# Anonymousijcai2024ttnet/scale_imagenet

Hardware: AMD Instinct MI355X
Metric: images/sec ImageNet 224x224, TT-small, MI355X; top-1 exact-match (higher is better)
Workload: dtype u16/u32/u64 packed bits (gate path); f32 as prescaled fp16x2 split operands on the 16-bit MFMA (stem, lin1, lin2); 1 GPU; TT_general_imagenet_v2_small forward, batch=256 224x224 per GPU, bit-packed HIP LUT kernels (BASELINE.json configs[1]); batch_per_gpu=256, global_batch=256, batches_in_flight=2, input=float32 NCHW, normalised (the reference's contract), parallelism=batch shard x1

## Files before the change

scale_imagenet_amd/csrc/gate_fused.hip:

```cpp

#include <type_traits>

#include "ttnet_common.h"

namespace ttnet {

namespace {

#ifndef TT_FUSED_SKIP
#define TT_FUSED_SKIP 0
#endif
constexpr int kSkip = TT_FUSED_SKIP;

constexpr int kFT = 1024;
constexpr int kFBuf = 65536;
constexpr int kFMaxScratch = 160 * 1024 - 2 * kFBuf;

template <int W>
using row_t = std::conditional_t<(W > 32), uint64_t, std::conditional_t<(W > 16), uint32_t, uint16_t>>;

template <int HO>
constexpr int fused_round() {
  constexpr int RG = (HO + 3) / 4, a = kFT / (16 * RG), b = kFMaxScratch / (HO * HO * 4);
  return a < b ? (a < 32 ? a : 32) : (b < 32 ? b : 32);
}

struct FusedArgs {
  int n, C, slices, off34, R;
  const void *x;
  const uint8_t *img_c3;
  const uint8_t *img_dw;
  const uint8_t *t_cf;
  void *y;
  uint32_t *idx;
};

__device__ inline void dma_table(uint8_t *dst, const uint8_t *src) {
  if constexpr (kSkip & 1) return;
  const int lane = threadIdx.x & 63, wave = threadIdx.x >> 6;
#pragma unroll
  for (int k = 0; k < kFBuf / 1024 / (kFT / 64); ++k) {
    const int chunk = wave + k * (kFT / 64);
    __builtin_amdgcn_global_load_lds((const __attribute__((address_space(1))) void *)(src + (size_t)chunk * 1024 + lane * 16),
                                     (__attribute__((address_space(3))) void *)(dst + chunk * 1024), 16, 0, 0);
  }
}

__device__ inline void phase_sync() {
  asm volatile("s_waitcnt vmcnt(0)" ::: "memory");
  __syncthreads();
}

__device__ inline uint32_t spread_nibbles(uint32_t x) {
  uint32_t y = (x | (x << 8)) & 0x00FF00FFu;
  return (y | (y << 4)) & 0x0F0F0F0Fu;
}

template <int WO, int OX0, int OX1>
__device__ inline void dw_lookup_pair(uint32_t pair, const uint8_t *tab, uint32_t c8, uint32_t &acc1, uint32_t &acc2) {
  if constexpr (OX0 < WO) {
    const uint2 w = *(const uint2 *)(tab + ((pair & 0xFFE0u) | c8));
    acc1 |= __builtin_amdgcn_ubfe(w.x, pair, 1) << OX0;
    acc2 |= __builtin_amdgcn_ubfe(w.y, pair, 1) << OX0;
  }
  if constexpr (OX1 < WO) {
    const uint32_t hi = pair >> 16;
    const uint2 w = *(const uint2 *)(tab + ((hi & 0xFFE0u) | c8));
    acc1 |= __builtin_amdgcn_ubfe(w.x, hi, 1) << OX1;
    acc2 |= __builtin_amdgcn_ubfe(w.y, hi, 1) << OX1;
  }
}

template <int WO, int OXB, int OXS>
__device__ inline void dw_eight(uint32_t R0, uint32_t R1, uint32_t R2, uint32_t R3, const uint8_t *tab, uint32_t c8,
                                uint32_t &acc1, uint32_t &acc2) {
  if constexpr (OXB >= WO) return;
  constexpr uint32_t M = 0x0F0F0F0Fu;
  const uint32_t t0 = (R0 & M) | ((R1 << 4) & ~M), u0 = (R2 & M) | ((R3 << 4) & ~M);
  dw_lookup_pair<WO, OXB, OXB + 2 * OXS>(__builtin_amdgcn_perm(u0, t0, 0x05010400u), tab, c8, acc1, acc2);
  dw_lookup_pair<WO, OXB + 4 * OXS, OXB + 6 * OXS>(__builtin_amdgcn_perm(u0, t0, 0x07030602u), tab, c8, acc1, acc2);
  if constexpr (OXB + OXS < WO) {
    const uint32_t t1 = ((R0 >> 4) & M) | (R1 & ~M), u1 = ((R2 >> 4) & M) | (R3 & ~M);
    dw_lookup_pair<WO, OXB + OXS, OXB + 3 * OXS>(__builtin_amdgcn_perm(u1, t1, 0x05010400u), tab, c8, acc1, acc2);
    dw_lookup_pair<WO, OXB + 5 * OXS, OXB + 7 * OXS>(__builtin_amdgcn_perm(u1, t1, 0x07030602u), tab, c8, acc1, acc2);
  }
}

template <int W, int WO>
__device__ inline void dw_row_both(const row_t<W> (&r)[4], const uint8_t *tab, uint32_t c8, uint32_t &acc1, uint32_t &acc2) {
  acc1 = 0;
  acc2 = 0;
  if constexpr (W > 32) {
    uint32_t plo[4], phi[4], qlo[4], qhi[4];
#pragma unroll
    for (int k = 0; k < 4; ++k) {
      qlo[k] = (uint32_t)r[k];
      qhi[k] = (uint32_t)((uint64_t)r[k] >> 32);
      plo[k] = qlo[k] << 2;
      phi[k] = __builtin_amdgcn_alignbit(qhi[k], qlo[k], 30);
    }
    dw_eight<WO, 0, 2>(plo[0], plo[1], plo[2], plo[3], tab, c8, acc1, acc2);
    dw_eight<WO, 16, 2>(phi[0], phi[1], phi[2], phi[3], tab, c8, acc1, acc2);
    dw_eight<WO, 1, 2>(qlo[0], qlo[1], qlo[2], qlo[3], tab, c8, acc1, acc2);
    dw_eight<WO, 17, 2>(qhi[0], qhi[1], qhi[2], qhi[3], tab, c8, acc1, acc2);
  } else {
    uint32_t p[4], q[4];
#pragma unroll
    for (int k = 0; k < 4; ++k) {
      q[k] = (uint32_t)r[k];
      p[k] = q[k] << 2;
    }
    dw_eight<WO, 0, 2>(p[0], p[1], p[2], p[3], tab, c8, acc1, acc2);
    dw_eight<WO, 1, 2>(q[0], q[1], q[2], q[3], tab, c8, acc1, acc2);
    static_assert(WO <= 16, "a 32-bit input row gives at most 16 output columns");
  }
}

__device__ inline uint32_t maj4_bytes(uint32_t v, uint32_t nb) {
  const uint32_t x = v & nb, y = v | nb;
  return (x | (x >> 8) | (y & (y >> 8))) & 0x00FF00FFu;
}

template <int H, int HO, bool LAST>
__global__ __launch_bounds__(kFT) void gate_block_kernel(FusedArgs a) {
  extern __shared__ __align__(16) uint8_t lds[];
  constexpr int W = H, WO = HO, HP = H / 2, WP = W / 2, PIX = HO * WO;
  constexpr int RG = (HO + 3) / 4;
  constexpr int LPR = WO <= 16 ? 16 : 32, RPW = 64 / LPR;
  using TI = row_t<W>;
  using TOut = row_t<WO>;
  uint8_t *const buf0 = lds, *const buf1 = lds + kFBuf;
  uint32_t *const S = (uint32_t *)(lds + 2 * kFBuf);

  const int strands = a.C / 8, P = strands / 2;
  int st, sl;
  {
    const int b = blockIdx.x, x = b & 7, k = b >> 3;
    if (P >= 8 && P % 8 == 0) {
      const int m = P / 8, pair = x + 8 * (k % m), kk = k / m;
      st = 2 * pair + (kk & 1);
      sl = kk >> 1;
    } else if (P == 4 && (a.slices & 1) == 0) {
      st = 2 * (x >> 1) + (k & 1);
      sl = (x & 1) * (a.slices / 2) + (k >> 1);
    } else {
      st = b % strands;
      sl = b / strands;
    }
  }
  const int n0 = (int)((long long)sl * a.n / a.slices), n1 = (int)((long long)(sl + 1) * a.n / a.slices);
  if (n0 >= n1) return;
  const int q = st >> 1, half = st & 1;
  const int tid0 = threadIdx.x, lane = tid0 & 63;
  const DwLaneConst lk = dw_lane_const(lane);
  auto opaque_tid = [&]() {
    int t = tid0;
    asm volatile("" : "+v"(t));
    return t;
  };
  const TI *const x = (const TI *)a.x;

  const uint8_t *const src_c3 = a.img_c3 + (size_t)st * kFBuf;
  const uint8_t *const src_dw0 = a.img_dw + (size_t)(2 * st) * kFBuf, *const src_dw1 = src_dw0 + kFBuf;
  const uint8_t *const src_cf0 = LAST ? nullptr : a.t_cf + (size_t)(2 * st) * kFBuf, *const src_cf1 = LAST ? nullptr : src_cf0 + kFBuf;

  constexpr int RMAX = fused_round<HO>();
  constexpr int TA = (RMAX * HP + kFT / 16 - 1) / (kFT / 16);
  static_assert(RMAX * RG * 16 <= kFT, "one depthwise task per thread");
  TI ra[TA][2];
  TI rb0[4], rb1[4];
  const int R = a.R;

  auto load_a = [&](int i0, int rn) {
    const int tid = opaque_tid();
    const int c = tid & 15, g = tid >> 4;
#pragma unroll
    for (int p = 0; p < TA; ++p) {
      const int gt = p * (kFT / 16) + g;
      const bool ok = gt < rn * HP;
      const int im = ok ? gt / HP : 0, py = ok ? gt - (gt / HP) * HP : 0;
      const TI *src = x + ((size_t)(n0 + i0 + im) * a.C + 16 * q + c) * H + 2 * py;
      ra[p][0] = ok ? src[0] : (TI)0;
      ra[p][1] = ok ? src[1] : (TI)0;
    }
  };
  auto load_b = [&](int i0, int rn, int sub, TI (&rb)[4]) {
    const int tid = opaque_tid();
    const int c4 = tid & 3, r = (tid >> 2) & 3, gi = tid >> 4;
    const int im = gi / RG, rg = gi - im * RG;
    const int oy = 4 * rg + r;
    const bool ok = im < rn && oy < HO;
    const TI *src = x + ((size_t)(n0 + i0 + (ok ? im : 0)) * a.C + 8 * st + 4 * sub + c4) * H;
#pragma unroll
    for (int kh = 0; kh < 4; ++kh) {
      const int iy = 2 * oy - 2 + kh;
      rb[kh] = (ok && iy >= 0 && iy < H) ? src[iy] : (TI)0;
    }
  };

  auto phase_a = [&](int rn, const uint8_t *tab) {
    if constexpr (kSkip & 2) return;
    const int tid = opaque_tid();
    for (int t = tid; t < rn * (HO + WO - 1); t += kFT) {
      const int im = t / (HO + WO - 1), e = t - im * (HO + WO - 1);
      const int edge = a.off34 ? 0 : HO - 1;
      const int pix = e < WO ? edge * WO + e : (e - WO + (a.off34 ? 1 : 0)) * WO + edge;
      *(uint16_t *)((uint8_t *)(S + im * PIX + pix) + 2) = 0;
    }
    const int g = tid >> 4, j = tid & 15;
    constexpr int CHUNKS = W > 32 ? 2 : 1, TPB = 2 / CHUNKS;
    static_assert(TA % TPB == 0, "phase A walks whole batches");
#pragma unroll
    for (int bt = 0; bt < TA / TPB; ++bt) {
      uint32_t d[4];
#pragma unroll
      for (int u = 0; u < 2; ++u) {
        const int p = bt * TPB + (CHUNKS == 2 ? 0 : u), k = CHUNKS == 2 ? u : 0;
        d[2 * u] = (uint32_t)((uint64_t)ra[p][0] >> (32 * k));
        d[2 * u + 1] = (uint32_t)((uint64_t)ra[p][1] >> (32 * k));
      }
      transpose16_multi<4>(d, lk);
      uint32_t v3[2], v4[2];
#pragma unroll
      for (int u = 0; u < 2; ++u) {
        const uint32_t t0 = d[2 * u], t1 = d[2 * u + 1];
        const uint32_t e00 = tab[t0 & 0xFFFFu], e01 = tab[t0 >> 16], e10 = tab[t1 & 0xFFFFu], e11 = tab[t1 >> 16];
        v3[u] = e00 | (e10 << 8) | (e01 << 16) | (e11 << 24);
        v4[u] = __builtin_amdgcn_perm(t1, t0, half ? 0x07030501u : 0x06020400u);
      }
      uint32_t n3[2], n4[2];
#pragma unroll
      for (int u = 0; u < 2; ++u) {
        n3[u] = lane_xor16<1>(v3[u]);
        n4[u] = lane_xor16<1>(v4[u]);
      }
#pragma unroll
      for (int u = 0; u < 2; ++u) {
        const int p = bt * TPB + (CHUNKS == 2 ? 0 : u), k = CHUNKS == 2 ? u : 0;
        const int gt = p * (kFT / 16) + g;
        const bool ok = gt < rn * HP;
        const int im = ok ? gt / HP : 0, py = ok ? gt - (gt / HP) * HP : 0;
        const uint32_t m3 = maj4_bytes(v3[u], n3[u]), m4 = maj4_bytes(v4[u], n4[u]);
        const uint32_t sh = (uint32_t)(j & 1) * 16u;
        const uint32_t t = ((m3 >> sh) & 0xFFu) | (((m4 >> sh) & 0xFFu) << 8);
        const uint32_t dlt = ((t >> 4) ^ t) & 0x00F0u;
        const uint32_t v = t ^ dlt ^ (dlt << 4);
        const int px = 16 * k + 8 * (j & 1) + (j >> 1);
        if (ok && px < WP) {
          const int pix = (py + a.off34) * WO + px + a.off34;
          *(uint16_t *)((uint8_t *)(S + im * PIX + pix) + 2) = (uint16_t)v;
        }
      }
      __builtin_amdgcn_sched_barrier(0);
    }
  };

  uint32_t bacc[2][2];
  auto phase_b_lookup = [&](const uint8_t *tab, int sub, const TI (&rb)[4]) {
    if constexpr (kSkip & 4) return;
    const int tid = opaque_tid();
    dw_row_both<W, WO>(rb, tab, (uint32_t)(tid & 3) * 8u, bacc[sub][0], bacc[sub][1]);
  };
  auto phase_b_store = [&](int rn) {
    if constexpr (kSkip & 4) return;
    const int tid = opaque_tid();
    const int j = tid & 15, gi = tid >> 4;
    const int im = gi / RG, rg = gi - im * RG;
    uint32_t t[4] = {bacc[0][0], bacc[0][1], bacc[1][0], bacc[1][1]};
    transpose16_multi<4>(t, lk);
    uint8_t *dst = (uint8_t *)(S + im * PIX + 4 * rg * WO + j);
    auto put = [&](uint32_t w0, uint32_t w1, int col0) {
      if (im < rn && col0 + j < WO) {
        const uint32_t lo = __builtin_amdgcn_perm(w1, w0, 0x05010400u), hi = __builtin_amdgcn_perm(w1, w0, 0x07030602u);
        if (4 * rg + 0 < HO) *(uint16_t *)(dst + (0 * WO + col0) * 4) = (uint16_t)lo;
        if (4 * rg + 1 < HO) *(uint16_t *)(dst + (1 * WO + col0) * 4) = (uint16_t)(lo >> 16);
        if (4 * rg + 2 < HO) *(uint16_t *)(dst + (2 * WO + col0) * 4) = (uint16_t)hi;
        if (4 * rg + 3 < HO) *(uint16_t *)(dst + (3 * WO + col0) * 4) = (uint16_t)(hi >> 16);
      }
    };
    put(spread_nibbles(t[0] & 0xFFFFu) | (spread_nibbles(t[1] & 0xFFFFu) << 4),
        spread_nibbles(t[2] & 0xFFFFu) | (spread_nibbles(t[3] & 0xFFFFu) << 4), 0);
    if constexpr (WO > 16)
      put(spread_nibbles(t[0] >> 16) | (spread_nibbles(t[1] >> 16) << 4), spread_nibbles(t[2] >> 16) | (spread_nibbles(t[3] >> 16) << 4), 16);
  };

  auto phase_c = [&](int i0, int rn, const uint8_t *tab, int kgrp) {
    if constexpr (kSkip & 8) return;
    const int tid = opaque_tid();
    const int lane = tid & 63, wave = __builtin_amdgcn_readfirstlane(tid >> 6);
    const int sub = lane / LPR, ox = lane % LPR;
    TOut *const y = (TOut *)a.y;
    constexpr int CH2 = (HO + 2 * RPW - 1) / (2 * RPW);
    constexpr int U = 2, NW = kFT / 64;
    const uint32_t sel = kgrp ? 0x0C0C0301u : 0x0C0C0200u;
    if (kgrp == 0 && a.idx)
      for (int t = tid; t < rn * PIX; t += kFT) a.idx[((size_t)(n0 + i0 + t / PIX) * strands + st) * PIX + (t % PIX)] = S[t];
    for (int wt0 = wave; wt0 < rn * CH2; wt0 += U * NW) {
      uint32_t w[U], d0[U], d1[U];
      int im[U], oy[U];
#pragma unroll
      for (int u = 0; u < U; ++u) {
        const int wt = wt0 + u * NW;
        im[u] = wt / CH2;
        oy[u] = (wt - im[u] * CH2) * 2 * RPW + sub;
        const bool live = wt < rn * CH2 && ox < WO;
        d0[u] = live && oy[u] < HO ? S[im[u] * PIX + oy[u] * WO + ox] : 0u;
        d1[u] = live && oy[u] + RPW < HO ? S[im[u] * PIX + (oy[u] + RPW) * WO + ox] : 0u;
      }
#pragma unroll
      for (int u = 0; u < U; ++u)
        w[u] = ox < WO ? (uint32_t)tab[__builtin_amdgcn_perm(0u, d0[u], sel)] | ((uint32_t)tab[__builtin_amdgcn_perm(0u, d1[u], sel)] << 8)
                       : 0u;
      transpose16_multi<U>(w, lk);
#pragma unroll
      for (int u = 0; u < U; ++u) {
        const uint32_t piece = w[u] & 0xFFFFu;
        uint32_t rowbits = piece;
        if constexpr (LPR == 32) rowbits |= (uint32_t)__shfl_xor((int)piece, 16) << 16;
        const int row = oy[u] + ((lane >> 3) & 1) * RPW;
        if (wt0 + u * NW < rn * CH2 && (lane & (LPR - 1)) < 16 && row < HO)
          y[((uint32_t)(n0 + i0 + im[u]) * (uint32_t)(2 * a.C) + 16 * st + 8 * kgrp + (lane & 7)) * HO + row] = (TOut)rowbits;
      }
    }
  };

  auto phase_out = [&](int i0, int rn) {
    const int tid = opaque_tid();
    for (int t = tid; t < rn * PIX; t += kFT)
      a.idx[((size_t)(n0 + i0 + t / PIX) * strands + st) * PIX + (t % PIX)] = S[t];
  };

  const int total = n1 - n0;
  int cur = 0;
  load_a(0, min(R, total));
  dma_table(buf0, src_c3);
  for (int i0 = 0; i0 < total; i0 += R) {
    const int rn = min(R, total - i0);
    const bool more = i0 + R < total;
    uint8_t *tb = cur ? buf1 : buf0, *nb = cur ? buf0 : buf1;
    phase_sync();
    load_b(i0, rn, 0, rb0);
    dma_table(nb, src_dw0);
    phase_a(rn, tb);
    cur ^= 1; tb = cur ? buf1 : buf0; nb = cur ? buf0 : buf1;
    phase_sync();
    load_b(i0, rn, 1, rb1);
    dma_table(nb, src_dw1);
    phase_b_lookup(tb, 0, rb0);
    cur ^= 1; tb = cur ? buf1 : buf0; nb = cur ? buf0 : buf1;
    phase_sync();
    if constexpr (LAST) {
      if (more) {
        load_a(i0 + R, min(R, total - i0 - R));
        dma_table(nb, src_c3);
      }
      phase_b_lookup(tb, 1, rb1);
      phase_b_store(rn);
      cur ^= 1;
      phase_sync();
      phase_out(i0, rn);
    } else {
      dma_table(nb, src_cf0);
      phase_b_lookup(tb, 1, rb1);
      phase_b_store(rn);
      cur ^= 1; tb = cur ? buf1 : buf0; nb = cur ? buf0 : buf1;
      phase_sync();
      dma_table(nb, src_cf1);
      phase_c(i0, rn, tb, 0);
      cur ^= 1; tb = cur ? buf1 : buf0; nb = cur ? buf0 : buf1;
      phase_sync();
      if (more) {
        load_a(i0 + R, min(R, total - i0 - R));
        dma_table(nb, src_c3);
      }
      phase_c(i0, rn, tb, 1);
      cur ^= 1;
    }
  }
}

__global__ void c3_image_kernel(const uint16_t *__restrict__ t_c3, uint8_t *__restrict__ img, int strands) {
  const size_t t = (size_t)blockIdx.x * blockDim.x + threadIdx.x;
  if (t >= (size_t)strands * 65536) return;
  const int st = (int)(t >> 16);
  const uint32_t idx = (uint32_t)(t & 0xFFFF);
  img[t] = (uint8_t)(t_c3[(size_t)(st >> 1) * 65536 + idx] >> (8 * (st & 1)));
}
__global__ void dw_image_kernel(const uint32_t *__restrict__ t1, const uint32_t *__restrict__ t2, uint32_t *__restrict__ img, int C) {
  const size_t t = (size_t)blockIdx.x * blockDim.x + threadIdx.x;
  if (t >= (size_t)C * 2048 * 2) return;
  const int br = (int)(t & 1), ch = (int)((t >> 1) & 3), row = (int)((t >> 3) & 2047), ss = (int)(t >> 14);
  const int channel = 4 * ss + ch;
  const uint32_t *src = br ? t2 : t1;
  img[t] = src[((size_t)(channel >> 4) * 2048 + row) * 16 + (channel & 15)];
}

__global__ void branch_rows_kernel(const uint32_t *__restrict__ idx, uint64_t *__restrict__ rows, int n, int C, int HO, int br) {
  const size_t t = (size_t)blockIdx.x * blockDim.x + threadIdx.x;
  if (t >= (size_t)n * C * HO) return;
  const int oy = (int)(t % HO), c = (int)((t / HO) % C), im = (int)(t / ((size_t)HO * C));
  const int st = c >> 3, k = c & 7;
  const int shift = 8 * ((br >> 1) * 2 + (k >> 2)) + 4 * (br & 1) + (k & 3);
  const uint32_t *src = idx + ((size_t)im * (C / 8) + st) * HO * HO + (size_t)oy * HO;
  uint64_t r = 0;
  for (int ox = 0; ox < HO; ++ox) r |= (uint64_t)((src[ox] >> shift) & 1u) << ox;
  rows[t] = r;
}
template <typename T>
__global__ void widen_rows_kernel(const T *__restrict__ src, uint64_t *__restrict__ dst, size_t count) {
  const size_t t = (size_t)blockIdx.x * blockDim.x + threadIdx.x;
  if (t < count) dst[t] = (uint64_t)src[t];
}
template <typename T>
__global__ void narrow_rows_kernel(const uint64_t *__restrict__ src, T *__restrict__ dst, size_t count) {
  const size_t t = (size_t)blockIdx.x * blockDim.x + threadIdx.x;
  if (t < count) dst[t] = (T)src[t];
}

template <int H, int HO, bool LAST>
int launch_block_t(const FusedBlockArgs &f, hipStream_t s) {
  auto k = gate_block_kernel<H, HO, LAST>;
  constexpr int PIX = HO * HO;
  const int strands = f.C / 8;
  int R = fused_round<HO>();
  const int slices = fused_block_slices(f.C, f.n);
  R = std::max(1, std::min(R, (f.n + slices - 1) / slices));
  const size_t lds = (size_t)2 * kFBuf + (size_t)R * PIX * 4;
  TT_TRY(ensure_dynamic_lds((const void *)k, kMaxLds));
  FusedArgs a{};
  a.n = f.n; a.C = f.C; a.slices = slices; a.off34 = f.off34; a.R = R;
  a.x = f.x; a.img_c3 = (const uint8_t *)f.img_c3; a.img_dw = (const uint8_t *)f.img_dw; a.t_cf = f.t_cf; a.y = f.y; a.idx = f.idx;
  hipLaunchKernelGGL(k, dim3(strands * slices), dim3(kFT), lds, s, a);
  TT_HIP(hipGetLastError());
  return TTNET_OK;
}

}

int row_bytes(int W) { return W > 32 ? 8 : (W > 16 ? 4 : 2); }

int fused_block_slices(int C, int n) {
  const int strands = C / 8;
  int slices = std::max(1, std::min(n, 256 / strands));
  if (strands == 8 && slices > 1 && (slices & 1)) slices -= 1;
  return slices;
}

bool fused_block_supported(int C, int H, int Ho, int stride, int pad, int kh, int kw) {
  if (stride != 2 || pad != 2 || kh != 4 || kw != 4 || C % 16) return false;
  return (H == 56 && Ho == 29) || (H == 29 && Ho == 15) || (H == 15 && Ho == 8) || (H == 8 && Ho == 5);
}

int launch_gate_block(const FusedBlockArgs &f, hipStream_t s) {
  if (f.last && !f.idx) {
    set_error("gate_block: a last block needs its branch-dword buffer");
    return TTNET_E_INVALID;
  }
#define TT_FUSED_CASE(h, ho)                                                         \
  if (f.H == h && f.Ho == ho) return f.last ? launch_block_t<h, ho, true>(f, s) : launch_block_t<h, ho, false>(f, s)
  if (f.H == 56 && f.Ho == 29 && !f.last) return launch_block_t<56, 29, false>(f, s);
  TT_FUSED_CASE(29, 15);
  TT_FUSED_CASE(15, 8);
  TT_FUSED_CASE(8, 5);
#undef TT_FUSED_CASE
  set_error("gate_block: no fused kernel for %dx%d -> %dx%d", f.H, f.H, f.Ho, f.Ho);
  return TTNET_E_UNSUPPORTED;
}

int launch_fused_images(const void *t_dw1, const void *t_dw2, const void *t_c3, int C, void *img_dw, void *img_c3, hipStream_t s) {
  {
    const size_t t = (size_t)(C / 8) * 65536;
    hipLaunchKernelGGL(c3_image_kernel, dim3((unsigned)((t + 255) / 256)), dim3(256), 0, s, (const uint16_t *)t_c3, (uint8_t *)img_c3,
                       C / 8);
  }
  {
    const size_t t = (size_t)C * 2048 * 2;
    hipLaunchKernelGGL(dw_image_kernel, dim3((unsigned)((t + 255) / 256)), dim3(256), 0, s, (const uint32_t *)t_dw1,
                       (const uint32_t *)t_dw2, (uint32_t *)img_dw, C);
  }
  TT_HIP(hipGetLastError());
  return TTNET_OK;
}

int launch_branch_rows(const uint32_t *idx, uint64_t *rows, int n, int C, int Ho, int branch, hipStream_t s) {
  const size_t t = (size_t)n * C * Ho;
  hipLaunchKernelGGL(branch_rows_kernel, dim3((unsigned)((t + 255) / 256)), dim3(256), 0, s, idx, rows, n, C, Ho, branch);
  TT_HIP(hipGetLastError());
  return TTNET_OK;
}

int launch_widen_rows(const void *src, uint64_t *dst, size_t count, int W, hipStream_t s) {
  const unsigned g = (unsigned)((count + 255) / 256);
  if (W > 32) hipLaunchKernelGGL(widen_rows_kernel<uint64_t>, dim3(g), dim3(256), 0, s, (const uint64_t *)src, dst, count);
  else if (W > 16) hipLaunchKernelGGL(widen_rows_kernel<uint32_t>, dim3(g), dim3(256), 0, s, (const uint32_t *)src, dst, count);
  else hipLaunchKernelGGL(widen_rows_kernel<uint16_t>, dim3(g), dim3(256), 0, s, (const uint16_t *)src, dst, count);
  TT_HIP(hipGetLastError());
  return TTNET_OK;
}

int launch_narrow_rows(const uint64_t *src, void *dst, size_t count, int W, hipStream_t s) {
  const unsigned g = (unsigned)((count + 255) / 256);
  if (W > 32) hipLaunchKernelGGL(narrow_rows_kernel<uint64_t>, dim3(g), dim3(256), 0, s, src, (uint64_t *)dst, count);
  else if (W > 16) hipLaunchKernelGGL(narrow_rows_kernel<uint32_t>, dim3(g), dim3(256), 0, s, src, (uint32_t *)dst, count);
  else hipLaunchKernelGGL(narrow_rows_kernel<uint16_t>, dim3(g), dim3(256), 0, s, src, (uint16_t *)dst, count);
  TT_HIP(hipGetLastError());
  return TTNET_OK;
}

}
```

scale_imagenet_amd/csrc/ttnet_common.h:

```cpp
#pragma once

#include <hip/hip_runtime.h>
#include <stdint.h>
#include <algorithm>
#include <string>
#include <type_traits>
#include <vector>

#include "../../include/ttnet.h"

namespace ttnet {

void set_error(const char *fmt, ...);

#define TT_HIP(call)                                                                       \
  do {                                                                                     \
    hipError_t e__ = (call);                                                               \
    if (e__ != hipSuccess) {                                                               \
      ::ttnet::set_error("%s failed: %s (%s:%d)", #call, hipGetErrorString(e__), __FILE__, \
                         __LINE__);                                                        \
      return TTNET_E_HIP;                                                                  \
    }                                                                                      \
  } while (0)

#define TT_TRY(expr)          \
  do {                        \
    int s__ = (expr);         \
    if (s__ != TTNET_OK) return s__; \
  } while (0)

constexpr int kWave = 64;
constexpr int kMaxLds = 160 * 1024;

struct BlockGeom {
  std::string name;
  int in_planes = 0, out_planes = 0, kh = 1, kw = 1, stride = 1, pad = 0, groups = 1;
  bool last = false;
  int cin_g() const { return in_planes / groups; }
  int mid_g() const { return 8 * in_planes / groups; }
  int cout_g() const { return out_planes / groups; }
  int nbits() const { return cin_g() * kh * kw; }
  int entry_bits() const { return last ? 32 * cout_g() : (cout_g() == 1 ? 1 : (cout_g() <= 8 ? 8 : 16)); }
  size_t table_bytes() const {
    size_t entries = (size_t)groups << nbits();
    if (last) return entries * cout_g() * sizeof(float);
    if (entry_bits() == 1) {
      const size_t per = ((size_t)1 << nbits()) / 8;
      return (size_t)groups * (per < 4 ? 4 : per);
    }
    return entries * entry_bits() / 8;
  }
};

#if defined(__HIPCC__)
template <int LANE>
__device__ inline void writelane64(uint32_t &lo, uint32_t &hi, uint64_t sval) {
  asm("s_nop 1\n\tv_writelane_b32 %0, %2, %4\n\tv_writelane_b32 %1, %3, %4"
      : "+v"(lo), "+v"(hi)
      : "s"((uint32_t)sval), "s"((uint32_t)(sval >> 32)), "n"(LANE));
}

template <int I, int N, typename F>
__device__ inline void static_for(F &&f) {
  if constexpr (I < N) {
    f(std::integral_constant<int, I>{});
    static_for<I + 1, N>(f);
  }
}

struct DwLaneConst {
  uint32_t c4;
  uint32_t rot[4];
  uint32_t keep[4];
};

__device__ inline DwLaneConst dw_lane_const(uint32_t lane) {
  DwLaneConst k;
  k.c4 = (lane & 15) << 2;
  constexpr uint32_t M[4] = {0x00FF00FFu, 0x0F0F0F0Fu, 0x33333333u, 0x55555555u};
  constexpr uint32_t S[4] = {8, 4, 2, 1};
#pragma unroll
  for (int i = 0; i < 4; ++i) {
    const bool low = (lane & S[i]) == 0;
    k.rot[i] = low ? 32 - S[i] : S[i];
    k.keep[i] = low ? M[i] : ~M[i];
  }
  return k;
}

__device__ inline uint32_t transpose16(uint32_t acc, const DwLaneConst &k) {
  constexpr int S[4] = {8, 4, 2, 1};
  static_for<0, 4>([&](auto i) {
    constexpr int I = decltype(i)::value;
    const uint32_t partner = (uint32_t)__builtin_amdgcn_ds_swizzle((int)acc, 0x1F | (S[I] << 10));
    const uint32_t moved = __builtin_amdgcn_alignbit(partner, partner, k.rot[I]);
    acc = moved ^ ((moved ^ acc) & k.keep[I]);
  });
  return acc;
}

template <int S>
__device__ inline uint32_t lane_xor16(uint32_t v) {
  static_assert(S == 8 || S == 4 || S == 2 || S == 1, "butterfly distances");
  if constexpr (S == 8) return (uint32_t)__builtin_amdgcn_mov_dpp((int)v, 0x128, 0xF, 0xF, true);
  else if constexpr (S == 4)
    return (uint32_t)__builtin_amdgcn_mov_dpp(__builtin_amdgcn_mov_dpp((int)v, 0x141, 0xF, 0xF, true), 0x1B, 0xF, 0xF, true);
  else if constexpr (S == 2) return (uint32_t)__builtin_amdgcn_mov_dpp((int)v, 0x4E, 0xF, 0xF, true);
  else return (uint32_t)__builtin_amdgcn_mov_dpp((int)v, 0xB1, 0xF, 0xF, true);
}

template <int N>
__device__ inline void transpose16_multi(uint32_t (&acc)[N], const DwLaneConst &k) {
  constexpr int S[4] = {8, 4, 2, 1};
  static_for<0, 4>([&](auto i) {
    constexpr int I = decltype(i)::value;
    uint32_t partner[N];
#pragma unroll
    for (int n = 0; n < N; ++n) partner[n] = lane_xor16<S[I]>(acc[n]);
#pragma unroll
    for (int n = 0; n < N; ++n) {
      const uint32_t moved = __builtin_amdgcn_alignbit(partner[n], partner[n], k.rot[I]);
      acc[n] = moved ^ ((moved ^ acc[n]) & k.keep[I]);
    }
  });
}

#endif

int ensure_dynamic_lds(const void *kernel, size_t bytes);


struct LutBuildArgs {
  const float *w1;
  const float *w2;
  const double *s1, *t1;
  const double *s2, *t2;
  const uint8_t *perm;
  int groups, n, mid_g, cout_g, last;
  void *table;
  unsigned *near_ties;
};
int launch_lut_build(const LutBuildArgs &a, hipStream_t s);

constexpr int SPLIT_PLANES = 2;
constexpr float ACT_PRESCALE = 16.0f;

__device__ inline void split_f16x2(float v, uint16_t &h1, uint16_t &h2) {
  const _Float16 a = (_Float16)v;
  const _Float16 b = (_Float16)(v - (float)a);
  h1 = __builtin_bit_cast(uint16_t, a);
  h2 = __builtin_bit_cast(uint16_t, b);
}
__device__ inline float f16_bits_to_float(uint16_t h) { return (float)__builtin_bit_cast(_Float16, h); }

__device__ inline bool split_out_of_range(float prescaled) { return !(__builtin_fabsf(prescaled) < 65504.0f); }

__device__ inline void store_feature(uint16_t *feat_frag, int img, int KS, int ks, int kk, float f, uint32_t *range_flag) {
  uint16_t h1, h2;
  const float fs = f * ACT_PRESCALE;
  if (split_out_of_range(fs)) *range_flag = 1u;
  split_f16x2(fs, h1, h2);
  const int ln = (img & 31) + 32 * (kk >> 3), j = kk & 7;
  const size_t base = ((size_t)(img >> 5) * KS + ks) * SPLIT_PLANES;
  feat_frag[((base + 0) * 64 + ln) * 8 + j] = h1;
  feat_frag[((base + 1) * 64 + ln) * 8 + j] = h2;
}
__device__ inline float load_feature(const uint16_t *feat_frag, int img, int KS, int ks, int kk) {
  const int ln = (img & 31) + 32 * (kk >> 3), j = kk & 7;
  const size_t base = ((size_t)(img >> 5) * KS + ks) * SPLIT_PLANES;
  return (f16_bits_to_float(feat_frag[((base + 1) * 64 + ln) * 8 + j]) + f16_bits_to_float(feat_frag[((base + 0) * 64 + ln) * 8 + j])) *
         (1.0f / ACT_PRESCALE);
}
float weight_prescale(const float *w, size_t n);

int launch_stem(const void *x, bool x_is_u8, const uint32_t *norm_tab, const void *wfrag, const float *init, uint64_t *rp,
                uint16_t *cp, int n, int p, uint32_t *range_flag, hipStream_t s, int workgroups = 0);
size_t stem_u8_table_elems();
bool stem_split_weights_u8(const float *w, const double *scale, const double *shift, int p, const float mean[3], const float stdv[3],
                           uint16_t *out, float *init, uint32_t *tab );
bool stem_split_weights(const float *w , const double *scale, const double *shift, int p, uint16_t *out,
                        float *init );
size_t stem_split_weights_elems();
int stem_kernel_arg_sizes(const int **sizes);

struct GateBlockArgs {
  int n;
  int C, H, W;
  int Ho, Wo;
  int off34;
  int kh1, kw1, kh2, kw2, stride, pad;
  int cf_bits;
  const uint64_t *x_rp;
  const uint16_t *x_cp;
  const uint8_t *t_dw1, *t_dw2;
  const uint16_t *t_c3;
  uint16_t *o1, *o2, *o3, *o4;
};
int launch_gate_stage1(const GateBlockArgs &a, hipStream_t s);
int gate_stage1_grid(int C, int n);
int launch_gate_pf(const GateBlockArgs &a, const uint8_t *t_cf, uint16_t *out_cp, uint64_t *out_rp, hipStream_t s);
int launch_gate_last(const GateBlockArgs &a, const float *t_last, void *feat_frag, uint32_t *range_flag, hipStream_t s,
                     const uint32_t *idx = nullptr);
struct FusedBlockArgs {
  int n, C, H, Ho, off34, last;
  const void *x;
  const void *img_c3, *img_dw;
  const uint8_t *t_cf;
  void *y;
  uint32_t *idx;
};
bool fused_block_supported(int C, int H, int Ho, int stride, int pad, int kh, int kw);
int row_bytes(int W);
int fused_block_slices(int C, int n);
int launch_gate_block(const FusedBlockArgs &f, hipStream_t s);
int launch_fused_images(const void *t_dw1, const void *t_dw2, const void *t_c3, int C, void *img_dw, void *img_c3, hipStream_t s);
int launch_branch_rows(const uint32_t *idx, uint64_t *rows, int n, int C, int Ho, int branch, hipStream_t s);
int launch_widen_rows(const void *src, uint64_t *dst, size_t count, int W, hipStream_t s);
int launch_narrow_rows(const uint64_t *src, void *dst, size_t count, int W, hipStream_t s);
int launch_xs_branches(const GateBlockArgs &a, const void *t_c3, uint64_t *const o[4], hipStream_t s);
int launch_xs_pf(int n, int C, int Ho, int Wo, int cout_g, uint64_t *const o[4], const void *t_cf, uint64_t *out_rp,
                 hipStream_t s);
int launch_xs_last(int n, int C, int Ho, int Wo, int cout_g, uint64_t *const o[4], const float *t_last, void *feat_frag,
                   uint32_t *range_flag, hipStream_t s);
struct FullDwArgs {
  int n, C, H, W;
  int kh, kw, stride, pad;
  int ho, wo;
  int Ho;
  int pad_t, pad_l;
  const uint64_t *x_rp;
  const float *w1, *w2;
  const double *s1, *t1, *s2, *t2;
  uint64_t *out;
  uint32_t *fix_list, *fix_count;
  uint32_t fix_cap;
  float tau_scale;
  const float *gel;
};
struct FullPwArgs {
  int n, H, W;
  int groups, cin, mid, cout, Cout;
  int Csrc;
  int interleaved;
  const uint64_t *src[4];
  const float *w1, *w2;
  const double *s1, *t1, *s2, *t2;
  uint64_t *out_rp;
  float *out_float;
  uint32_t *fix_list, *fix_count, *range_flag;
  float tau_scale;
  const float *gel;
};
int launch_full_dw(const FullDwArgs &a, hipStream_t s);
int launch_full_pw(const FullPwArgs &a, hipStream_t s);
size_t full_gelu_tables_elems();
int launch_full_gelu_tables(float *dst, hipStream_t s);
int launch_rp_majority(const uint64_t *x, uint64_t *out, int n, int C, int H, int W, int Ho, int pad_t, int pad_l,
                       hipStream_t s);
int launch_full_pool_split(const float *x, void *feat_frag, int n, int C, int H, int W, uint32_t *range_flag, hipStream_t s);
int launch_va_stem(const float *x, const float *w, const float *bias, const float *scale, const float *shift,
                   uint64_t *rp, int n, hipStream_t s);
int launch_va_block(const uint64_t *x_rp, const void *t1, const void *t2, const void *t3, uint64_t *y, int n, hipStream_t s);
int launch_va_feat(const uint64_t *y, void *feat_frag, int n, hipStream_t s);
int launch_va_frag_to_flat(const void *af, float *out, int n, hipStream_t s);
int launch_cp_to_rp(const uint16_t *cp, uint64_t *rp, int n, int C, int H, int W, hipStream_t s);
int launch_rp_to_cp(const uint64_t *rp, uint16_t *cp, int n, int C, int H, int W, hipStream_t s);
int launch_frag_to_reference_order(const void *af, float *out, int n, int G, int PP, hipStream_t s);
int gemm_f16x2_splits(int M, int N, int KS);
size_t gemm_f16x2_part_elems(int M, int N, int KS);
int launch_gemm_f16x2(const void *Af, const void *Bf, float *part, int M, int N, int K, int splits, hipStream_t s);
size_t frag_elems(int rows, int K);
int launch_split_to_frag(const float *src, void *dst, int R, int K, int rows_padded, float prescale, hipStream_t s, int ld = 0,
                         int kvalid = 0);

int launch_head_mid(const float *part, int splits, const float *scale, const float *shift, void *mid_frag, int M, int N,
                    int polynomial, uint32_t *range_flag, hipStream_t s);
int launch_lin2_f16x2(const void *mid_frag, const void *w2f, const float *bias, float inv, float *out, int M, int N, int K,
                      hipStream_t s);
int launch_permute_lin1(const float *w1, float *w1p, int O, int G, int PP, hipStream_t s);

constexpr int kUsagePlain = 0, kUsageMerged = 1;
int launch_usage_dw(const uint64_t *x_rp, int n, int C, int H, int W, int Ho, int Wo, int kh, int kw, int stride, int pad,
                    int64_t *counters, int scheme, hipStream_t s);
int launch_usage_pw(const uint64_t *const *src, int nsrc, int n, int Csrc, int groups, int cin_g, int H, int W, int64_t *counters,
                    int scheme, hipStream_t s);

}
```

Before: 1.971 million images/s.

## Repack depthwise LUT as 16-bit interleaved branches and use raw LDS addressing

Result: faster. 2.026 million images/s (median of 6 runs) (+2.8%).

```diff
diff --git a/scale_imagenet_amd/csrc/gate_fused.hip b/scale_imagenet_amd/csrc/gate_fused.hip
--- a/scale_imagenet_amd/csrc/gate_fused.hip
+++ b/scale_imagenet_amd/csrc/gate_fused.hip
@@ -51,45 +51,51 @@
   __syncthreads();
 }
 
+typedef const __attribute__((address_space(3))) uint8_t *lds_bytes_t;
+__device__ inline uint32_t lds_addr(const void *p) { return (uint32_t)(uintptr_t)(lds_bytes_t)p; }
+__device__ inline uint32_t lds_read_u8(uint32_t addr) { return *(lds_bytes_t)(uintptr_t)addr; }
+__device__ inline uint32_t lds_read_u32(uint32_t addr) { return *(const __attribute__((address_space(3))) uint32_t *)(uintptr_t)addr; }
+
 __device__ inline uint32_t spread_nibbles(uint32_t x) {
   uint32_t y = (x | (x << 8)) & 0x00FF00FFu;
   return (y | (y << 4)) & 0x0F0F0F0Fu;
 }
 
+typedef uint16_t u16x2 __attribute__((ext_vector_type(2)));
+
 template <int WO, int OX0, int OX1>
-__device__ inline void dw_lookup_pair(uint32_t pair, const uint8_t *tab, uint32_t c8, uint32_t &acc1, uint32_t &acc2) {
+__device__ inline void dw_lookup_pair(uint32_t pair, uint32_t base, uint32_t &acc) {
+  constexpr uint32_t P0 = OX0 & 15, P1 = OX1 & 15;
+  const uint32_t adj = __builtin_bit_cast(uint32_t, __builtin_bit_cast(u16x2, pair) - __builtin_bit_cast(u16x2, P0 | (P1 << 16)));
   if constexpr (OX0 < WO) {
-    const uint2 w = *(const uint2 *)(tab + ((pair & 0xFFE0u) | c8));
-    acc1 |= __builtin_amdgcn_ubfe(w.x, pair, 1) << OX0;
-    acc2 |= __builtin_amdgcn_ubfe(w.y, pair, 1) << OX0;
+    const uint32_t w = lds_read_u32((pair & 0xFFF0u) | base);
+    acc |= __builtin_amdgcn_alignbit(w, w, adj) & (0x00010001u << P0);
   }
   if constexpr (OX1 < WO) {
-    const uint32_t hi = pair >> 16;
-    const uint2 w = *(const uint2 *)(tab + ((hi & 0xFFE0u) | c8));
-    acc1 |= __builtin_amdgcn_ubfe(w.x, hi, 1) << OX1;
-    acc2 |= __builtin_amdgcn_ubfe(w.y, hi, 1) << OX1;
+    const uint32_t w = lds_read_u32(((pair >> 16) & 0xFFF0u) | base);
+    acc |= __builtin_amdgcn_alignbit(w, w, adj >> 16) & (0x00010001u << P1);
   }
 }
 
 template <int WO, int OXB, int OXS>
-__device__ inline void dw_eight(uint32_t R0, uint32_t R1, uint32_t R2, uint32_t R3, const uint8_t *tab, uint32_t c8,
-                                uint32_t &acc1, uint32_t &acc2) {
+__device__ inline void dw_eight(uint32_t R0, uint32_t R1, uint32_t R2, uint32_t R3, uint32_t base, uint32_t &acc) {
   if constexpr (OXB >= WO) return;
+  static_assert((OXB >> 4) == ((OXB + 7 * OXS) >> 4), "one accumulator per 16 columns");
   constexpr uint32_t M = 0x0F0F0F0Fu;
   const uint32_t t0 = (R0 & M) | ((R1 << 4) & ~M), u0 = (R2 & M) | ((R3 << 4) & ~M);
-  dw_lookup_pair<WO, OXB, OXB + 2 * OXS>(__builtin_amdgcn_perm(u0, t0, 0x05010400u), tab, c8, acc1, acc2);
-  dw_lookup_pair<WO, OXB + 4 * OXS, OXB + 6 * OXS>(__builtin_amdgcn_perm(u0, t0, 0x07030602u), tab, c8, acc1, acc2);
+  dw_lookup_pair<WO, OXB, OXB + 2 * OXS>(__builtin_amdgcn_perm(u0, t0, 0x05010400u), base, acc);
+  dw_lookup_pair<WO, OXB + 4 * OXS, OXB + 6 * OXS>(__builtin_amdgcn_perm(u0, t0, 0x07030602u), base, acc);
   if constexpr (OXB + OXS < WO) {
     const uint32_t t1 = ((R0 >> 4) & M) | (R1 & ~M), u1 = ((R2 >> 4) & M) | (R3 & ~M);
-    dw_lookup_pair<WO, OXB + OXS, OXB + 3 * OXS>(__builtin_amdgcn_perm(u1, t1, 0x05010400u), tab, c8, acc1, acc2);
-    dw_lookup_pair<WO, OXB + 5 * OXS, OXB + 7 * OXS>(__builtin_amdgcn_perm(u1, t1, 0x07030602u), tab, c8, acc1, acc2);
+    dw_lookup_pair<WO, OXB + OXS, OXB + 3 * OXS>(__builtin_amdgcn_perm(u1, t1, 0x05010400u), base, acc);
+    dw_lookup_pair<WO, OXB + 5 * OXS, OXB + 7 * OXS>(__builtin_amdgcn_perm(u1, t1, 0x07030602u), base, acc);
   }
 }
 
 template <int W, int WO>
-__device__ inline void dw_row_both(const row_t<W> (&r)[4], const uint8_t *tab, uint32_t c8, uint32_t &acc1, uint32_t &acc2) {
-  acc1 = 0;
-  acc2 = 0;
+__device__ inline void dw_row_both(const row_t<W> (&r)[4], uint32_t base, uint32_t &accl, uint32_t &acch) {
+  accl = 0;
+  acch = 0;
   if constexpr (W > 32) {
     uint32_t plo[4], phi[4], qlo[4], qhi[4];
 #pragma unroll
@@ -99,10 +105,10 @@
       plo[k] = qlo[k] << 2;
       phi[k] = __builtin_amdgcn_alignbit(qhi[k], qlo[k], 30);
     }
-    dw_eight<WO, 0, 2>(plo[0], plo[1], plo[2], plo[3], tab, c8, acc1, acc2);
-    dw_eight<WO, 16, 2>(phi[0], phi[1], phi[2], phi[3], tab, c8, acc1, acc2);
-    dw_eight<WO, 1, 2>(qlo[0], qlo[1], qlo[2], qlo[3], tab, c8, acc1, acc2);
-    dw_eight<WO, 17, 2>(qhi[0], qhi[1], qhi[2], qhi[3], tab, c8, acc1, acc2);
+    dw_eight<WO, 0, 2>(plo[0], plo[1], plo[2], plo[3], base, accl);
+    dw_eight<WO, 16, 2>(phi[0], phi[1], phi[2], phi[3], base, acch);
+    dw_eight<WO, 1, 2>(qlo[0], qlo[1], qlo[2], qlo[3], base, accl);
+    dw_eight<WO, 17, 2>(qhi[0], qhi[1], qhi[2], qhi[3], base, acch);
   } else {
     uint32_t p[4], q[4];
 #pragma unroll
@@ -110,8 +116,8 @@
       q[k] = (uint32_t)r[k];
       p[k] = q[k] << 2;
     }
-    dw_eight<WO, 0, 2>(p[0], p[1], p[2], p[3], tab, c8, acc1, acc2);
-    dw_eight<WO, 1, 2>(q[0], q[1], q[2], q[3], tab, c8, acc1, acc2);
+    dw_eight<WO, 0, 2>(p[0], p[1], p[2], p[3], base, accl);
+    dw_eight<WO, 1, 2>(q[0], q[1], q[2], q[3], base, accl);
     static_assert(WO <= 16, "a 32-bit input row gives at most 16 output columns");
   }
 }
@@ -131,6 +137,7 @@
   using TOut = row_t<WO>;
   uint8_t *const buf0 = lds, *const buf1 = lds + kFBuf;
   uint32_t *const S = (uint32_t *)(lds + 2 * kFBuf);
+  if (lds_addr(lds) & (kFBuf - 1)) __builtin_trap();
 
   const int strands = a.C / 8, P = strands / 2;
   int st, sl;
@@ -208,6 +215,7 @@
       *(uint16_t *)((uint8_t *)(S + im * PIX + pix) + 2) = 0;
     }
     const int g = tid >> 4, j = tid & 15;
+    const uint32_t tb = lds_addr(tab);
     constexpr int CHUNKS = W > 32 ? 2 : 1, TPB = 2 / CHUNKS;
     static_assert(TA % TPB == 0, "phase A walks whole batches");
 #pragma unroll
@@ -224,7 +232,8 @@
 #pragma unroll
       for (int u = 0; u < 2; ++u) {
         const uint32_t t0 = d[2 * u], t1 = d[2 * u + 1];
-        const uint32_t e00 = tab[t0 & 0xFFFFu], e01 = tab[t0 >> 16], e10 = tab[t1 & 0xFFFFu], e11 = tab[t1 >> 16];
+        const uint32_t e00 = lds_read_u8((t0 & 0xFFFFu) | tb), e01 = lds_read_u8(__builtin_amdgcn_alignbit(tb >> 16, t0, 16));
+        const uint32_t e10 = lds_read_u8((t1 & 0xFFFFu) | tb), e11 = lds_read_u8(__builtin_amdgcn_alignbit(tb >> 16, t1, 16));
         v3[u] = e00 | (e10 << 8) | (e01 << 16) | (e11 << 24);
         v4[u] = __builtin_amdgcn_perm(t1, t0, half ? 0x07030501u : 0x06020400u);
       }
@@ -259,15 +268,21 @@
   auto phase_b_lookup = [&](const uint8_t *tab, int sub, const TI (&rb)[4]) {
     if constexpr (kSkip & 4) return;
     const int tid = opaque_tid();
-    dw_row_both<W, WO>(rb, tab, (uint32_t)(tid & 3) * 8u, bacc[sub][0], bacc[sub][1]);
+    dw_row_both<W, WO>(rb, lds_addr(tab) | (uint32_t)(tid & 3) * 4u, bacc[sub][0], bacc[sub][1]);
   };
   auto phase_b_store = [&](int rn) {
     if constexpr (kSkip & 4) return;
     const int tid = opaque_tid();
     const int j = tid & 15, gi = tid >> 4;
     const int im = gi / RG, rg = gi - im * RG;
-    uint32_t t[4] = {bacc[0][0], bacc[0][1], bacc[1][0], bacc[1][1]};
-    transpose16_multi<4>(t, lk);
+    constexpr int NT = WO > 16 ? 4 : 2;
+    uint32_t t[NT];
+    if constexpr (WO > 16) {
+      t[0] = bacc[0][0]; t[1] = bacc[1][0]; t[2] = bacc[0][1]; t[3] = bacc[1][1];
+    } else {
+      t[0] = bacc[0][0]; t[1] = bacc[1][0];
+    }
+    transpose16_multi<NT>(t, lk);
     uint8_t *dst = (uint8_t *)(S + im * PIX + 4 * rg * WO + j);
     auto put = [&](uint32_t w0, uint32_t w1, int col0) {
       if (im < rn && col0 + j < WO) {
@@ -278,10 +293,9 @@
         if (4 * rg + 3 < HO) *(uint16_t *)(dst + (3 * WO + col0) * 4) = (uint16_t)(hi >> 16);
       }
     };
-    put(spread_nibbles(t[0] & 0xFFFFu) | (spread_nibbles(t[1] & 0xFFFFu) << 4),
-        spread_nibbles(t[2] & 0xFFFFu) | (spread_nibbles(t[3] & 0xFFFFu) << 4), 0);
+    put(spread_nibbles(t[0] & 0xFFFFu) | (spread_nibbles(t[0] >> 16) << 4), spread_nibbles(t[1] & 0xFFFFu) | (spread_nibbles(t[1] >> 16) << 4), 0);
     if constexpr (WO > 16)
-      put(spread_nibbles(t[0] >> 16) | (spread_nibbles(t[1] >> 16) << 4), spread_nibbles(t[2] >> 16) | (spread_nibbles(t[3] >> 16) << 4), 16);
+      put(spread_nibbles(t[2] & 0xFFFFu) | (spread_nibbles(t[2] >> 16) << 4), spread_nibbles(t[3] & 0xFFFFu) | (spread_nibbles(t[3] >> 16) << 4), 16);
   };
 
   auto phase_c = [&](int i0, int rn, const uint8_t *tab, int kgrp) {
@@ -292,7 +306,8 @@
     TOut *const y = (TOut *)a.y;
     constexpr int CH2 = (HO + 2 * RPW - 1) / (2 * RPW);
     constexpr int U = 2, NW = kFT / 64;
-    const uint32_t sel = kgrp ? 0x0C0C0301u : 0x0C0C0200u;
+    const uint32_t sel = kgrp ? 0x05040301u : 0x05040200u;
+    const uint32_t tbh = lds_addr(tab) >> 16;
     if (kgrp == 0 && a.idx)
       for (int t = tid; t < rn * PIX; t += kFT) a.idx[((size_t)(n0 + i0 + t / PIX) * strands + st) * PIX + (t % PIX)] = S[t];
     for (int wt0 = wave; wt0 < rn * CH2; wt0 += U * NW) {
@@ -309,7 +324,7 @@
       }
 #pragma unroll
       for (int u = 0; u < U; ++u)
-        w[u] = ox < WO ? (uint32_t)tab[__builtin_amdgcn_perm(0u, d0[u], sel)] | ((uint32_t)tab[__builtin_amdgcn_perm(0u, d1[u], sel)] << 8)
+        w[u] = ox < WO ? lds_read_u8(__builtin_amdgcn_perm(tbh, d0[u], sel)) | (lds_read_u8(__builtin_amdgcn_perm(tbh, d1[u], sel)) << 8)
                        : 0u;
       transpose16_multi<U>(w, lk);
 #pragma unroll
@@ -389,10 +404,11 @@
 __global__ void dw_image_kernel(const uint32_t *__restrict__ t1, const uint32_t *__restrict__ t2, uint32_t *__restrict__ img, int C) {
   const size_t t = (size_t)blockIdx.x * blockDim.x + threadIdx.x;
   if (t >= (size_t)C * 2048 * 2) return;
-  const int br = (int)(t & 1), ch = (int)((t >> 1) & 3), row = (int)((t >> 3) & 2047), ss = (int)(t >> 14);
-  const int channel = 4 * ss + ch;
-  const uint32_t *src = br ? t2 : t1;
-  img[t] = src[((size_t)(channel >> 4) * 2048 + row) * 16 + (channel & 15)];
+  const int ch = (int)(t & 3), d = (int)((t >> 2) & 4095), ss = (int)(t >> 14);
+  const int channel = 4 * ss + ch, row = d >> 1, up = d & 1;
+  const size_t src = ((size_t)(channel >> 4) * 2048 + row) * 16 + (channel & 15);
+  const uint32_t h1 = (t1[src] >> (16 * up)) & 0xFFFFu, h2 = (t2[src] >> (16 * up)) & 0xFFFFu;
+  img[t] = up ? (h1 << 16) | h2 : h1 | (h2 << 16);
 }
 
 __global__ void branch_rows_kernel(const uint32_t *__restrict__ idx, uint64_t *__restrict__ rows, int n, int C, int HO, int br) {
diff --git a/scale_imagenet_amd/csrc/ttnet_common.h b/scale_imagenet_amd/csrc/ttnet_common.h
--- a/scale_imagenet_amd/csrc/ttnet_common.h
+++ b/scale_imagenet_amd/csrc/ttnet_common.h
@@ -94,7 +94,7 @@
     constexpr int I = decltype(i)::value;
     const uint32_t partner = (uint32_t)__builtin_amdgcn_ds_swizzle((int)acc, 0x1F | (S[I] << 10));
     const uint32_t moved = __builtin_amdgcn_alignbit(partner, partner, k.rot[I]);
-    acc = moved ^ ((moved ^ acc) & k.keep[I]);
+    acc = __builtin_amdgcn_bitop3_b32(k.keep[I], acc, moved, 0xCA);
   });
   return acc;
 }
@@ -120,7 +120,7 @@
 #pragma unroll
     for (int n = 0; n < N; ++n) {
       const uint32_t moved = __builtin_amdgcn_alignbit(partner[n], partner[n], k.rot[I]);
-      acc[n] = moved ^ ((moved ^ acc[n]) & k.keep[I]);
+      acc[n] = __builtin_amdgcn_bitop3_b32(k.keep[I], acc[n], moved, 0xCA);
     }
   });
 }
```
